# Blaizzy/mlx-audio

Measured on AMD Instinct MI355X. Metric: audio samples/sec + real-time factor, Kokoro-82M TTS, higher is better.
Workload: dtype bf16 weights x fp32 activations: vocoder convs = fp16 hi pass (v_mfma_f32_32x32x16_f16) + block-scaled FP4 (e2m1) lo pass (v_mfma_scale_f32_32x32x64_f8f6f4 cbsz / blgp 4, OCP MX: E8M0 scale per row x 32 channels / per output column), fp32 accumulate; front end bf16 hi+lo split; 1 GPU; Kokoro-82M bf16 TTS, tokens->waveform, canonical short sentence T=80 F=264 (6.6 s @ 24 kHz); utterances_per_gpu=64, global_batch=64, samples_per_utterance=158400, parallelism=utterance-dp1, precision_mode=6, wire=fp32

## Files before the change

include/mi355audio.h:

```cpp
#ifndef MI355AUDIO_H
#define MI355AUDIO_H

#include <stdint.h>

#ifdef __cplusplus
extern "C" {
#endif

#define MI355_OK 0
#define MI355_ERR_ARG (-1)
#define MI355_ERR_LAUNCH (-2)
#define MI355_ERR_UNSUPPORTED (-3)

const char* mi355_last_error(void);
int mi355_abi_version(void);
int mi355_device_info(int dev, char* name, int name_cap, int* cu_count, int* lds_bytes);

enum { MI355_ACT_NONE = 0, MI355_ACT_LEAKY = 1, MI355_ACT_SNAKE = 2, MI355_ACT_GELU = 3,
       MI355_ACT_ELU = 4,
       MI355_ACT_SILU = 5,
       MI355_ACT_GELU_TANH = 6,
       MI355_ACT_TANH = 7 };

typedef struct {
// ... 265 lines not shown
  int32_t pre_tanh;
  float* y; int64_t y_bstride; int32_t ldy;
  int32_t B; int32_t T; int32_t C; int32_t pad;
} mi355_ecapa_rows_args;
int mi355_ecapa_rows(const mi355_ecapa_rows_args* a, void* stream);
typedef struct {
  const float* x; int64_t x_bstride; int32_t ldx;
  int32_t B; int32_t T; int32_t C;
  float eps;
  float* mean; float* std; int32_t out_ld;
} mi355_time_moments_args;
int mi355_time_moments(const mi355_time_moments_args* a, void* stream);
typedef struct {
  const float* x; int64_t x_bstride; int32_t ldx;
  const float* logits; int64_t l_bstride; int32_t ldl;
  int32_t B; int32_t T; int32_t C;
  float eps;
  float* out; int32_t out_ld;
} mi355_attentive_pool_args;
int mi355_attentive_pool(const mi355_attentive_pool_args* a, void* stream);

typedef struct {
  const float* x; int64_t x_bstride; int32_t ldx; int32_t C; int32_t L; const int32_t* lens; int32_t B;
  const float* up_filter; const float* down_filter;
  const float* alpha; const float* inv_beta;
  float* y; int64_t y_bstride; int32_t ldy;
} mi355_aa_act_args;
int mi355_aa_activation(const mi355_aa_act_args* a, void* stream);

typedef struct {
  const float* x; int64_t x_bstride; int32_t n_in; int32_t rows;
  const double* table; int32_t up; int32_t down; int32_t K; int32_t first;
  float* y; int64_t y_bstride; int32_t n_out;
} mi355_resample_args;
int mi355_resample_poly(const mi355_resample_args* a, void* stream);

typedef struct {
  const float* x; int64_t x_bstride; int32_t ldx; int32_t C; int32_t L; const int32_t* lens; int32_t B;
  const float* scale; const float* shift; int32_t pre_ld; float slope;
  const float* w;
  const float* bias;
  float* y; int64_t y_bstride; int32_t ldy;
} mi355_pool_up2_args;
int mi355_adain_pool_up2(const mi355_pool_up2_args* a, void* stream);

typedef struct {
  const float* x; int64_t x_rstride; int32_t W; int64_t rows;
  int32_t size; int32_t mode; int32_t align_corners; float scale; float half_scale;
  float* y; int64_t y_rstride;
} mi355_interp1d_args;
int mi355_interpolate1d(const mi355_interp1d_args* a, void* stream);

int mi355_conv1d_c1_k3s2(const float* x, int32_t ldx_b, int32_t Lin, const int32_t* lens_in,
                         float w0, float w1, float w2, float bias, float* y, int64_t y_bstride, int32_t ldy, int32_t col,
                         int32_t Lout, int32_t B, void* stream);

typedef struct {
  const float* f0; int32_t ld_f0; int32_t L2; const int32_t* lens2; int32_t B;
  int32_t up; int32_t H; float sr; float sine_amp; float noise_std; float voiced_thr;
  const float* rand_ini; const float* noise;
  const float* lin_w; float lin_b;
  float* phase_ws;
  float* out; int32_t ld_out;
  float* quant_ws;
  int32_t coarse_f32;
} mi355_sine_source_args;
int mi355_sine_source(const mi355_sine_source_args* a, void* stream);

typedef struct {
  const float* x; int32_t ldx; int32_t L; const int32_t* lens; int32_t B;
  int32_t n_fft; int32_t hop; const float* window;
  float* y; int64_t y_bstride; int32_t ldy;
} mi355_stft_magphase_args;
int mi355_stft_magphase(const mi355_stft_magphase_args* a, void* stream);

typedef struct {
  const float* x; int64_t x_bstride; int32_t ldx; int32_t Fr; const int32_t* lens; int32_t B;
  int32_t n_fft; int32_t hop; const float* window;
  float* audio; int32_t ld_audio;
} mi355_istft_head_args;
int mi355_istft_head(const mi355_istft_head_args* a, void* stream);

typedef struct {
  const float* x; int32_t ldx; int32_t L; int32_t B;
  int32_t n_fft; int32_t hop; const float* window;
  int32_t pad_mode; int32_t n_frames;
  float* out;
} mi355_stft_args;
int mi355_stft(const mi355_stft_args* a, void* stream);

typedef struct {
  const float* x; int32_t ldx; int32_t L; int32_t B;
  int32_t n_fft; int32_t hop; const float* window; int32_t pad_mode; int32_t n_frames;
  const float* fb; int32_t n_mels; int32_t mode;
  float* out;
  float* gmax;
  float log_guard;
} mi355_logmel_args;
int mi355_logmel(const mi355_logmel_args* a, void* stream);
int mi355_logmel_finish(float* y, int64_t n_per_item, const float* gmax, int32_t B, void* stream);

typedef struct {
  const float* x; int32_t L;
  int32_t win; int32_t shift; int32_t pad; int32_t n_fft; int32_t n_frames;
  const float* window;
  const float* noise;
  float dither; float preemph;
  float* frames;
} mi355_kaldi_frames_args;
int mi355_kaldi_frames(const mi355_kaldi_frames_args* a, void* stream);
int mi355_polar_spec(const float* x, int64_t x_bstride, int32_t ldx, int32_t Fr, int32_t nb, int32_t B, float clip, float* spec, void* stream);


typedef struct {
  const float* spec; int32_t n_frames; int32_t B;
  int32_t n_fft; int32_t hop; const float* window; const float* norm;
  int32_t norm_mode;
  int32_t clamp; int32_t trim; int32_t out_len;
  float* frames_ws;
  float* out; int32_t ld_out;
} mi355_istft_args;
int mi355_istft(const mi355_istft_args* a, void* stream);

enum { MI355_KV_F32 = 0, MI355_KV_BF16 = 1, MI355_KV_F16 = 2 };
typedef struct {
  const float* q; int64_t q_bstride; int32_t ldq;
  const float* k; int64_t k_bstride; int32_t ldk;
  const float* v; int64_t v_bstride; int32_t ldv;
  int32_t heads; int32_t kv_heads; int32_t dh;
  int32_t Tq; int32_t Tk;
  const int32_t* lens_q;
  const int32_t* lens_k;
  int32_t causal; int32_t window; float scale;
  int32_t B;
  int32_t mode;
  float* out; int64_t out_bstride; int32_t ldo;
  const int32_t* k_start;
  float* split_ws; int32_t* split_cnt; int32_t nsplit;
  int64_t k_hstride; int64_t v_hstride;
  int32_t kv_dtype;
  const float* new_k; const float* new_v; int64_t new_bstride;
  const float* q_norm_w; const float* k_norm_w; float norm_eps;
  const float* rope_cos; const float* rope_sin; int32_t rope_rows; int32_t rope_mode; int32_t rope_pos;
  int32_t in_kgroups; int64_t in_kg_stride; const float* q_bias; const float* k_bias; const float* v_bias;
  const float* q_wscale; const float* k_wscale; const float* v_wscale;
  uint16_t* out_planes; int32_t planes_R; int32_t planes_dtype;
} mi355_flash_attn_args;
int mi355_flash_attention(const mi355_flash_attn_args* a, void* stream);

typedef struct {
  const float* logits; int32_t ld; int32_t V; int32_t B;
  int32_t* tokens; int32_t tokens_ld; int32_t n;
  int32_t sample_begin;
  const float* suppress_mask;
  const int32_t* blank_ids; int32_t n_blank;
  int32_t timestamp_rules;
  int32_t timestamp_begin; int32_t eot; int32_t no_timestamps;
  int32_t max_initial_timestamp_index;
  const float* gumbel; float temperature;
  float* sum_logprobs;
  float* filtered;
  const int32_t* forced_next;
  float* split_ws; int32_t* split_cnt;
} mi355_whisper_step_args;
int mi355_whisper_greedy_step(const mi355_whisper_step_args* a, void* stream);
int mi355_softmax_prob_at(const float* logits, int32_t ld, int32_t V, int32_t B, int32_t token, float* out, void* stream);
// ... 284 lines not shown
```

mlx_audio_amd/csrc/source.hip:

```cpp
#include "block_reduce.h"

namespace {

#pragma clang fp contract(off)

__device__ __forceinline__ float mul_rn(float a, float b) { return a * b; }
__device__ __forceinline__ float add_rn(float a, float b) { return a + b; }
__device__ __forceinline__ float sub_rn(float a, float b) { return a - b; }

__device__ __forceinline__ void lin_coord(int i, float scale, float half_scale, int in_w, int& lo, int& hi, float& fr) {
  float x = mul_rn((float)i, scale);
  x = add_rn(x, half_scale);
  x = sub_rn(x, 0.5f);
  x = fmaxf(x, 0.0f);
  lo = (int)floorf(x);
  hi = min(lo + 1, in_w - 1);
  fr = sub_rn(x, (float)lo);
}

struct SineDims { int L; int small; int big; float sc_dn, hsc_dn, sc_up, hsc_up; };

__host__ __device__ inline SineDims sine_dims(int len2, int up, int coarse_f32) {
  SineDims d;
  d.L = len2 * up;
// ... 194 lines not shown
    const int j = i / N, n = i - j * N;
    const float* sp = spec + j * nb * 2;
    double acc = (double)sp[0];
    if ((N & 1) == 0) acc += ((n & 1) ? -1.0 : 1.0) * (double)sp[(nb - 1) * 2];
    const int kend = (N & 1) ? nb : nb - 1;
    int m = n;
    for (int k = 1; k < kend; ++k) {
      acc += 2.0 * ((double)sp[k * 2] * twc[m] - (double)sp[k * 2 + 1] * tws[m]);
      m += n; if (m >= N) m -= N;
    }
    td[i] = mul_rn((float)(acc / (double)N), win[n]);
  }
  __syncthreads();
  const int total = (Fr - 1) * hop;
  for (int i = threadIdx.x; i < kHeadFrames * hop; i += blockDim.x) {
    const int p = blockIdx.x * kHeadFrames * hop + i;
    const int t = p - N / 2;
    if (t < 0 || t >= total) continue;
    int f_lo = (p - N + hop) / hop; if (p - N + 1 <= 0) f_lo = 0;
    int f_hi = p / hop; if (f_hi > Fr - 1) f_hi = Fr - 1;
    float rec = 0.f, ws = 0.f;
    for (int f = f_lo; f <= f_hi; ++f) {
      const int n = p - f * hop;
      if (n < 0 || n >= N) continue;
      rec = add_rn(rec, td[(f - fa) * N + n]);
      ws = add_rn(ws, mul_rn(win[n], win[n]));
    }
    a.audio[(int64_t)b * a.ld_audio + t] = (ws > 1e-10f) ? rec / ws : rec;
  }
}

struct SmallTw { double c[32]; double s[32]; };

template <int N, int HOP>
__global__ __launch_bounds__(256) void stft_magphase_fast_kernel(const mi355_stft_magphase_args a, const SmallTw tw) {
  constexpr int nb = N / 2 + 1, FB = 256, SPAN = (FB - 1) * HOP + N, YS = 2 * nb + 1;
  __shared__ float xs[SPAN];
  __shared__ float ys[FB * YS];
  const int b = blockIdx.y, tid = threadIdx.x;
  const int len = a.lens ? a.lens[b] : a.L;
  const int nframes = len / HOP + 1;
  const int f0 = blockIdx.x * FB;
  if (f0 >= nframes) return;
  const float* xb = a.x + (int64_t)b * a.ldx;
  for (int j = tid; j < SPAN; j += 256) {
    int i = f0 * HOP + j - N / 2;
    if (i < 0) i = -i;
    if (i >= len) i = 2 * (len - 1) - i;
    i = i < 0 ? 0 : (i >= len ? len - 1 : i);
    xs[j] = xb[i];
  }
  __syncthreads();
  double xw[N];
#pragma unroll
  for (int n = 0; n < N; ++n) xw[n] = (double)mul_rn(xs[tid * HOP + n], a.window[n]);
  double sp[N / 2], sm[N / 2];
#pragma unroll
  for (int n = 1; n < N / 2; ++n) { sp[n] = xw[n] + xw[N - n]; sm[n] = xw[n] - xw[N - n]; }
  float* yrow = ys + tid * YS;
#pragma unroll
  for (int k = 0; k < nb; ++k) {
    double re = (k & 1) ? xw[0] - xw[N / 2] : xw[0] + xw[N / 2];
    double im = 0.0;
#pragma unroll
    for (int n = 1; n < N / 2; ++n) {
      const int m = (k * n) % N;
      re = fma(sp[n], tw.c[m], re);
      im = fma(-sm[n], tw.s[m], im);
    }
    const float ref = (float)re;
    const float imf = (k == 0 || 2 * k == N) ? 0.0f : (float)im;
    yrow[k] = hypotf(ref, imf);
    yrow[nb + k] = atan2f(imf, ref);
  }
  __syncthreads();
  float* yb = a.y + (int64_t)b * a.y_bstride;
  const int nrows = min(FB, nframes - f0);
  for (int i = tid; i < nrows * 2 * nb; i += 256) {
    const int r = i / (2 * nb), c = i - r * (2 * nb);
    yb[(int64_t)(f0 + r) * a.ldy + c] = ys[r * YS + c];
  }
}

template <int N, int HOP>
__global__ __launch_bounds__(256) void istft_head_fast_kernel(const mi355_istft_head_args a, const SmallTw tw) {
  constexpr int nb = N / 2 + 1, HALO = (N + HOP - 1) / HOP, FT = 256, FO = FT - HALO, XS = 2 * nb + 1, TS = N + 1;
  __shared__ float xin[FT * XS];
  __shared__ float td[FT * TS];
  const int b = blockIdx.y, tid = threadIdx.x;
  const int Fr = a.lens ? a.lens[b] : a.Fr;
  const int fa = blockIdx.x * FO - HALO;
  const float* xb = a.x + (int64_t)b * a.x_bstride;
  for (int i = tid; i < FT * 2 * nb; i += 256) {
    const int j = i / (2 * nb), c = i - j * (2 * nb), f = fa + j;
    xin[j * XS + c] = (f >= 0 && f < Fr) ? xb[(int64_t)f * a.ldx + c] : 0.f;
  }
  __syncthreads();
  {
    const int f = fa + tid;
    const bool valid = f >= 0 && f < Fr;
    const float* xr = xin + tid * XS;
    double re[nb], im[nb];
#pragma unroll
    for (int k = 0; k < nb; ++k) {
      const float mag = expf(xr[k]);
      const float ph = sinf(xr[nb + k]);
      float sn, cs;
      sincosf(ph, &sn, &cs);
      re[k] = valid ? (double)mul_rn(mag, cs) : 0.0;
      im[k] = valid ? (double)mul_rn(mag, sn) : 0.0;
    }
    float* tr = td + tid * TS;
#pragma unroll
    for (int n = 0; n <= N / 2; ++n) {
      const double base = (n & 1) ? re[0] - re[nb - 1] : re[0] + re[nb - 1];
      double A = 0.0, Bs = 0.0;
#pragma unroll
      for (int k = 1; k < nb - 1; ++k) {
        const int m = (k * n) % N;
        A = fma(re[k], tw.c[m], A);
        Bs = fma(im[k], tw.s[m], Bs);
      }
      constexpr double inv_n = 1.0 / (double)N;
      tr[n] = mul_rn((float)((base + 2.0 * (A - Bs)) * inv_n), a.window[n]);
      if (n > 0 && n < N / 2) tr[N - n] = mul_rn((float)((base + 2.0 * (A + Bs)) * inv_n), a.window[N - n]);
    }
  }
  __syncthreads();
  const int total = (Fr - 1) * HOP;
  for (int i = tid; i < FO * HOP; i += 256) {
    const int p = blockIdx.x * FO * HOP + i;
    const int t = p - N / 2;
    if (t < 0 || t >= total) continue;
    int f_lo = (p - N + HOP) / HOP; if (p - N + 1 <= 0) f_lo = 0;
    int f_hi = p / HOP; if (f_hi > Fr - 1) f_hi = Fr - 1;
    float rec = 0.f, ws = 0.f;
    for (int f = f_lo; f <= f_hi; ++f) {
      const int n = p - f * HOP;
      if (n < 0 || n >= N) continue;
      rec = add_rn(rec, td[(f - fa) * TS + n]);
      const float w = a.window[n];
      ws = add_rn(ws, mul_rn(w, w));
    }
    a.audio[(int64_t)b * a.ld_audio + t] = (ws > 1e-10f) ? rec / ws : rec;
  }
}

SmallTw make_small_tw(int N) {
  SmallTw tw;
  for (int m = 0; m < 32; ++m) {
    const long double ang = 2.0L * 3.14159265358979323846264338327950288L * (long double)(m % N) / (long double)N;
    tw.c[m] = (double)cosl(ang);
    tw.s[m] = (double)sinl(ang);
  }
  for (int m = 0; m < N; ++m) {
    if ((4 * m) % N == 0) {
      const int q = (4 * m) / N;
      tw.c[m] = q == 0 ? 1.0 : (q == 2 ? -1.0 : 0.0);
      tw.s[m] = q == 1 ? 1.0 : (q == 3 ? -1.0 : 0.0);
    }
  }
  return tw;
}

__global__ __launch_bounds__(256) void interpolate1d_kernel(const mi355_interp1d_args a) {
  const int64_t i = (int64_t)blockIdx.x * 256 + threadIdx.x;
  if (i >= a.rows * (int64_t)a.size) return;
  const int64_t r = i / a.size;
  const int o = (int)(i - r * a.size);
  const float* xr = a.x + r * a.x_rstride;
  float* yr = a.y + r * a.y_rstride;
  const int W = a.W;
  if (a.mode == 0) {
    int idx = a.size == 1 ? 0 : (int)floorf(((float)o * a.scale));
    idx = idx < 0 ? 0 : (idx > W - 1 ? W - 1 : idx);
    yr[o] = xr[idx];
    return;
  }
  if (W == 1) { yr[o] = xr[0]; return; }
  float x;
  if (a.align_corners && a.size > 1) x = ((float)o * a.scale);
  else if (a.size == 1) x = 0.f;
  else {
    x = ((float)o * a.scale);
    if (!a.align_corners) {
      x = x + a.half_scale;
      x = x - 0.5f;
      x = fmaxf(x, 0.f);
    }
  }
  const int lo = (int)floorf(x);
  const int hi = lo + 1 < W - 1 ? lo + 1 : W - 1;
  const float frac = x - (float)lo;
  const float lo_term = xr[lo < W ? lo : W - 1] * (1.0f - frac);
  const float hi_term = xr[hi] * frac;
  yr[o] = lo_term + hi_term;
}

__device__ __forceinline__ float fq_prologue(const mi355_fake_quant_args& a, float t, int b, int c) {
  if (a.pre_scale) t = t * a.pre_scale[(int64_t)b * a.pre_ld + c] + a.pre_shift[(int64_t)b * a.pre_ld + c];
  if (a.pre_act == MI355_ACT_LEAKY) t = t > 0.f ? t : t * a.pre_slope;
  else if (a.pre_act == MI355_ACT_SNAKE) {
    const float al = a.pre_alpha[c];
    const float sn = sinf(al * t);
    t = t + (1.0f / al) * (sn * sn);
  }
  return t;
}

template <bool VEC>
__global__ __launch_bounds__(256) void fq_prepare_kernel(const mi355_fake_quant_args a) {
  const int b = blockIdx.y;
  const int len = a.lens ? a.lens[b] : a.L;
  const float* xb = a.x + (int64_t)b * a.x_bstride;
  float* yb = a.y + (int64_t)b * a.y_bstride;
  float nmn = 0.f, mx = 0.f;
  if (VEC) {
    const int C4 = a.C >> 2, rps = C4 >= 256 ? 1 : 256 / C4, span = C4 >= 256 ? 256 : C4;
    const int ty = C4 >= 256 ? 0 : (int)threadIdx.x / C4, tx = (int)threadIdx.x - ty * span;
    for (int l = blockIdx.x * rps + ty; l < len && ty < rps; l += gridDim.x * rps) {
      for (int c4 = tx; c4 < C4; c4 += span) {
        const float4 v = *(const float4*)(xb + (int64_t)l * a.ldx + 4 * c4);
        float4 t;
        t.x = fq_prologue(a, v.x, b, 4 * c4);
        t.y = fq_prologue(a, v.y, b, 4 * c4 + 1);
        t.z = fq_prologue(a, v.z, b, 4 * c4 + 2);
        t.w = fq_prologue(a, v.w, b, 4 * c4 + 3);
        *(float4*)(yb + (int64_t)l * a.ldy + 4 * c4) = t;
// ... 60 lines not shown
  MI355_CLEAR_ERROR();
  if (vec) {
    const int c4 = a.C / 4, rps = c4 >= 256 ? 1 : 256 / c4;
    const unsigned nblk = (unsigned)std::max<int64_t>(1, std::min<int64_t>(((int64_t)a.L + 8 * rps - 1) / (8 * rps), 4096 / std::max(1, a.B) + 1));
    hipLaunchKernelGGL(fq_prepare_kernel<true>, dim3(nblk, a.B), dim3(256), 0, st, a);
    MI355_LAUNCH_CHECK("fake_quant_u8 (prepare)");
    hipLaunchKernelGGL(fq_apply_kernel<true>, dim3(nblk, a.B), dim3(256), 0, st, a);
    MI355_LAUNCH_CHECK("fake_quant_u8 (apply)");
    return MI355_OK;
  }
  const unsigned nblk = (unsigned)std::min<int64_t>((n + 1023) / 1024, 1024);
  hipLaunchKernelGGL(fq_prepare_kernel<false>, dim3(nblk, a.B), dim3(256), 0, st, a);
  MI355_LAUNCH_CHECK("fake_quant_u8 (prepare)");
  hipLaunchKernelGGL(fq_apply_kernel<false>, dim3(nblk, a.B), dim3(256), 0, st, a);
  MI355_LAUNCH_CHECK("fake_quant_u8 (apply)");
  return MI355_OK;
}

extern "C" int mi355_sine_source(const mi355_sine_source_args* ap, void* stream) {
  MI355_REQUIRE(ap && ap->f0 && ap->rand_ini && ap->noise && ap->lin_w && ap->phase_ws && ap->out, "sine_source: null tensor");
  const mi355_sine_source_args a = *ap;
  MI355_REQUIRE(a.H > 0 && a.H <= 64 && a.up > 0 && a.L2 > 0 && a.B > 0, "sine_source: bad shape");
  const SineDims d = sine_dims(a.L2, a.up, a.coarse_f32);
  MI355_REQUIRE(d.small <= a.L2 + 1, "sine_source: coarse length %d exceeds workspace", d.small);
  hipStream_t st = (hipStream_t)stream;
  MI355_CLEAR_ERROR();
  MI355_REQUIRE(a.H <= kMergeMaxH, "sine_source: at most %d harmonics", kMergeMaxH);
  hipLaunchKernelGGL(sine_phase_kernel, dim3(a.B), dim3(256), sizeof(float) * a.H * kPhaseChunk, st, a);
  MI355_LAUNCH_CHECK("sine_phase");
  MI355_CLEAR_ERROR();
  if (a.quant_ws) {
    hipError_t e = hipMemsetAsync(a.quant_ws, 0, sizeof(float) * 2 * a.B, st);
    MI355_REQUIRE(e == hipSuccess, "sine_source: memset failed: %s", hipGetErrorString(e));
    hipLaunchKernelGGL(sine_merge_kernel<true>, dim3((d.L + 255) / 256, a.B), dim3(256), 0, st, a);
    MI355_LAUNCH_CHECK("sine_merge (extrema)");
  }
  hipLaunchKernelGGL(sine_merge_kernel<false>, dim3((d.L + 255) / 256, a.B), dim3(256), 0, st, a);
  MI355_LAUNCH_CHECK("sine_merge");
  return MI355_OK;
}

extern "C" int mi355_stft_magphase(const mi355_stft_magphase_args* ap, void* stream) {
  MI355_REQUIRE(ap && ap->x && ap->window && ap->y, "stft_magphase: null tensor");
  const mi355_stft_magphase_args a = *ap;
  MI355_REQUIRE(a.n_fft >= 2 && a.n_fft <= kMaxSmallFft, "stft_magphase: n_fft must be in [2, %d]", kMaxSmallFft);
  MI355_REQUIRE(a.hop > 0 && a.L > a.n_fft / 2, "stft_magphase: input too short for reflect padding");
  const int nframes = a.L / a.hop + 1;
  MI355_CLEAR_ERROR();
  if (a.n_fft == 20 && a.hop == 5) {
    static const SmallTw tw20 = make_small_tw(20);
    hipLaunchKernelGGL((stft_magphase_fast_kernel<20, 5>), dim3((nframes + 255) / 256, a.B), dim3(256), 0, (hipStream_t)stream, a, tw20);
    MI355_LAUNCH_CHECK("stft_magphase");
    return MI355_OK;
  }
  hipLaunchKernelGGL(stft_magphase_kernel, dim3((nframes + 255) / 256, a.B), dim3(256), 0, (hipStream_t)stream, a);
  MI355_LAUNCH_CHECK("stft_magphase");
  return MI355_OK;
}

extern "C" int mi355_istft_head(const mi355_istft_head_args* ap, void* stream) {
  MI355_REQUIRE(ap && ap->x && ap->window && ap->audio, "istft_head: null tensor");
  const mi355_istft_head_args a = *ap;
  MI355_REQUIRE(a.n_fft >= 2 && a.n_fft <= kMaxSmallFft && a.hop > 0 && a.Fr > 1, "istft_head: bad shape");
  const int N = a.n_fft, nb = N / 2 + 1;
  if (N == 20 && a.hop == 5) {
    static const SmallTw tw20 = make_small_tw(20);
    constexpr int FO = 256 - (20 + 5 - 1) / 5;
    const int total_untrimmed = (a.Fr - 1) * 5 + 20;
    MI355_CLEAR_ERROR();
    hipLaunchKernelGGL((istft_head_fast_kernel<20, 5>), dim3((total_untrimmed + FO * 5 - 1) / (FO * 5), a.B), dim3(256), 0, (hipStream_t)stream, a, tw20);
    MI355_LAUNCH_CHECK("istft_head");
    return MI355_OK;
  }
  const int halo = (N + a.hop - 1) / a.hop, FT = kHeadFrames + halo;
  const size_t lds = sizeof(double) * 2 * N + sizeof(float) * N + sizeof(float) * FT * nb * 2 + sizeof(float) * FT * N;
  const int total_untrimmed = (a.Fr - 1) * a.hop + N;
  const int blocks = (total_untrimmed + kHeadFrames * a.hop - 1) / (kHeadFrames * a.hop);
  MI355_CLEAR_ERROR();
  hipLaunchKernelGGL(istft_head_kernel, dim3(blocks, a.B), dim3(256), lds, (hipStream_t)stream, a);
  MI355_LAUNCH_CHECK("istft_head");
  return MI355_OK;
}

extern "C" int mi355_interpolate1d(const mi355_interp1d_args* ap, void* stream) {
  MI355_REQUIRE(ap && ap->x && ap->y, "interpolate1d: null tensor");
  const mi355_interp1d_args a = *ap;
  MI355_REQUIRE(a.rows > 0 && a.W >= 1 && a.size >= 1 && (a.mode == 0 || a.mode == 1), "interpolate1d: bad arguments");
  MI355_CLEAR_ERROR();
  const int64_t n = a.rows * (int64_t)a.size;
  hipLaunchKernelGGL(interpolate1d_kernel, dim3((unsigned)((n + 255) / 256)), dim3(256), 0, (hipStream_t)stream, a);
  MI355_LAUNCH_CHECK("interpolate1d");
  return MI355_OK;
}
```

mlx_audio_amd/ops.py:

```python
from __future__ import annotations

import ctypes
import math
import os
from dataclasses import dataclass
from typing import Optional, Tuple

import numpy as np
import torch

from . import _lib

ACT_NONE, ACT_LEAKY, ACT_SNAKE, ACT_GELU, ACT_ELU, ACT_SILU, ACT_GELU_TANH, ACT_TANH = 0, 1, 2, 3, 4, 5, 6, 7

PROFILE = None


def _stream() -> int:
    return torch.cuda.current_stream().cuda_stream


def profile_finalize(entries):
    torch.cuda.synchronize()
    out = []
# ... 1285 lines not shown
    raw = torch.zeros((B, T), dtype=torch.float32, device=device)
    frames = torch.empty((B,), dtype=torch.int32, device=device)
    idx = torch.zeros((B, idx_cap), dtype=torch.int32, device=device)
    kw = dict(T=T, lens=_ptr(lens), B=B, speed=speed, forced_dur=_ptr(forced), dur=_ptr(dur), dur_raw=_ptr(raw),
              frames=_ptr(frames), idx=_ptr(idx), idx_ld=idx_cap, bins=bins, max_frames=max_frames)
    if logits is not None:
        _, _, _, bs, ld = _nlc(logits)
        kw.update(logits=_ptr(logits), bstride=bs, ld=ld)
    _lib.call_struct("mi355_duration_align", "mi355_duration_args", _stream(), **kw)
    return dur, raw, frames, idx


def adain_pool_up2(x: torch.Tensor, scale, shift, slope: float, w: torch.Tensor, bias: torch.Tensor, y: torch.Tensor, lens=None):
    B, L, C, xbs, ldx = _nlc(x)
    _, _, _, ybs, ldy = _nlc(y)
    _lib.call_struct("mi355_adain_pool_up2", "mi355_pool_up2_args", _stream(), x=_ptr(x), x_bstride=xbs, ldx=ldx, C=C, L=L,
                     lens=_ptr(lens), B=B, scale=_ptr(scale), shift=_ptr(shift), pre_ld=scale.stride(0), slope=slope,
                     w=_ptr(w), bias=_ptr(bias), y=_ptr(y), y_bstride=ybs, ldy=ldy)
    return y


def aa_activation(x: torch.Tensor, y: torch.Tensor, up_filter: torch.Tensor, down_filter: torch.Tensor, alpha: torch.Tensor, inv_beta: torch.Tensor, lens=None):
    B, L, C, xbs, ldx = _nlc(x)
    _, _, _, ybs, ldy = _nlc(y)
    assert up_filter.numel() == 12 and down_filter.numel() == 12 and alpha.numel() >= C and inv_beta.numel() >= C
    _lib.call_struct("mi355_aa_activation", "mi355_aa_act_args", _stream(), x=_ptr(x), x_bstride=xbs, ldx=ldx, C=C, L=L, lens=_ptr(lens), B=B,
                     up_filter=_ptr(up_filter), down_filter=_ptr(down_filter), alpha=_ptr(alpha), inv_beta=_ptr(inv_beta), y=_ptr(y), y_bstride=ybs, ldy=ldy)
    return y


def resample_poly(x: torch.Tensor, table: torch.Tensor, up: int, down: int, first: int, n_out: int, y: Optional[torch.Tensor] = None) -> torch.Tensor:
    assert x.dim() == 2 and x.dtype == torch.float32 and x.stride(1) == 1 and table.dtype == torch.float64 and table.is_contiguous() and table.shape[1] == up
    rows, n_in = x.shape
    if y is None:
        y = torch.empty(rows, n_out, device=x.device, dtype=torch.float32)
    assert y.shape == (rows, n_out) and y.stride(1) == 1 and y.dtype == torch.float32
    _lib.call_struct("mi355_resample_poly", "mi355_resample_args", _stream(), x=_ptr(x), x_bstride=x.stride(0), n_in=n_in, rows=rows, table=_ptr(table),
                     up=up, down=down, K=table.shape[0], first=first, y=_ptr(y), y_bstride=y.stride(0), n_out=n_out)
    return y


def conv1d_c1_k3s2(x: torch.Tensor, w3, bias: float, y: torch.Tensor, col: int, lens_in=None):
    assert x.dim() == 2 and x.stride(1) == 1
    B, Lout, _, ybs, ldy = _nlc(y)
    lib = _lib.load()
    rc = lib.mi355_conv1d_c1_k3s2(_ptr(x), x.stride(0), x.shape[1], _ptr(lens_in), float(w3[0]), float(w3[1]), float(w3[2]),
                                  float(bias), _ptr(y), ybs, ldy, col, Lout, B, _stream())
    _lib.check(rc, "mi355_conv1d_c1_k3s2")
    return y


def sine_source(f0: torch.Tensor, rand_ini: torch.Tensor, noise: torch.Tensor, lin_w: torch.Tensor, lin_b: float, up: int,
                lens2=None, sr: float = 24000.0, sine_amp: float = 0.1, noise_std: float = 0.003, voiced_thr: float = 10.0, quant: bool = False,
                coarse_f32: bool = False):
    B, L2 = f0.shape
    H = rand_ini.shape[1]
    assert f0.stride(1) == 1 and noise.is_contiguous() and tuple(noise.shape) == (B, L2 * up, H)
    ws = torch.empty((B, H, L2 + 1), dtype=torch.float32, device=f0.device)
    out = torch.zeros((B, L2 * up), dtype=torch.float32, device=f0.device)
    _lib.call_struct("mi355_sine_source", "mi355_sine_source_args", _stream(), f0=_ptr(f0), ld_f0=f0.stride(0), L2=L2,
                     lens2=_ptr(lens2), B=B, up=up, H=H, sr=sr, sine_amp=sine_amp, noise_std=noise_std, voiced_thr=voiced_thr,
                     rand_ini=_ptr(rand_ini), noise=_ptr(noise), lin_w=_ptr(lin_w), lin_b=lin_b, phase_ws=_ptr(ws),
                     out=_ptr(out), ld_out=out.stride(0),
                     quant_ws=_ptr(torch.empty((B, 2), dtype=torch.float32, device=f0.device)) if quant else None, coarse_f32=int(bool(coarse_f32)))
    return out


def stft_magphase(x: torch.Tensor, n_fft: int, hop: int, window: torch.Tensor, y: torch.Tensor, lens=None):
    assert x.dim() == 2 and x.stride(1) == 1
    B, _, _, ybs, ldy = _nlc(y)
    _lib.call_struct("mi355_stft_magphase", "mi355_stft_magphase_args", _stream(), x=_ptr(x), ldx=x.stride(0), L=x.shape[1],
                     lens=_ptr(lens), B=B, n_fft=n_fft, hop=hop, window=_ptr(window), y=_ptr(y), y_bstride=ybs, ldy=ldy)
    return y


def istft_head(x: torch.Tensor, n_fft: int, hop: int, window: torch.Tensor, audio: torch.Tensor, lens=None):
    B, Fr, _, xbs, ldx = _nlc(x)
    _lib.call_struct("mi355_istft_head", "mi355_istft_head_args", _stream(), x=_ptr(x), x_bstride=xbs, ldx=ldx, Fr=Fr,
                     lens=_ptr(lens), B=B, n_fft=n_fft, hop=hop, window=_ptr(window), audio=_ptr(audio),
                     ld_audio=audio.stride(0))
    return audio


def stft_frames(x: torch.Tensor, n_fft: int, hop: int, window: torch.Tensor, pad_mode: int, n_frames: int):
    assert x.dim() == 2 and x.stride(1) == 1 and x.dtype == torch.float32
    B, L = x.shape
    out = torch.empty((B, n_frames, n_fft // 2 + 1, 2), dtype=torch.float32, device=x.device)
    _lib.call_struct("mi355_stft", "mi355_stft_args", _stream(), x=_ptr(x), ldx=x.stride(0), L=L, B=B, n_fft=n_fft, hop=hop,
                     window=_ptr(window), pad_mode=pad_mode, n_frames=n_frames, out=_ptr(out))
    return torch.view_as_complex(out)


def logmel(x: torch.Tensor, n_fft: int, hop: int, window: torch.Tensor, pad_mode: int, n_frames: int, fb: torch.Tensor,
           mode: int, log_guard: float = 0.0, fixed_max: Optional[float] = None):
    assert x.dim() == 2 and x.stride(1) == 1 and fb.is_contiguous()
    B, L = x.shape
    n_mels = fb.shape[0]
    out = torch.empty((B, n_frames, n_mels), dtype=torch.float32, device=x.device)
    gmax = torch.empty((B,), dtype=torch.float32, device=x.device) if mode == 0 else None
    _lib.call_struct("mi355_logmel", "mi355_logmel_args", _stream(), x=_ptr(x), ldx=x.stride(0), L=L, B=B, n_fft=n_fft,
                     hop=hop, window=_ptr(window), pad_mode=pad_mode, n_frames=n_frames, fb=_ptr(fb), n_mels=n_mels,
                     mode=mode, out=_ptr(out), gmax=None if fixed_max is not None else _ptr(gmax), log_guard=float(log_guard))
    if mode == 0:
        if fixed_max is not None:
            gmax.fill_(float(fixed_max))
        lib = _lib.load()
        rc = lib.mi355_logmel_finish(_ptr(out), n_frames * n_mels, _ptr(gmax), B, _stream())
        _lib.check(rc, "mi355_logmel_finish")
    return out


def kaldi_frames(x: torch.Tensor, win: int, shift: int, pad: int, n_fft: int, n_frames: int, window: torch.Tensor, preemph: float,
                 noise: Optional[torch.Tensor] = None, dither: float = 0.0) -> torch.Tensor:
    assert x.dim() == 1 and x.is_contiguous() and x.dtype == torch.float32 and window.numel() == win
    out = torch.empty((n_frames, n_fft), dtype=torch.float32, device=x.device)
    if noise is not None:
        assert noise.is_contiguous() and tuple(noise.shape) == (n_frames, win)
    _lib.call_struct("mi355_kaldi_frames", "mi355_kaldi_frames_args", _stream(), x=_ptr(x), L=x.numel(), win=win, shift=shift, pad=pad, n_fft=n_fft,
                     n_frames=n_frames, window=_ptr(window), noise=_ptr(noise), dither=dither, preemph=preemph, frames=_ptr(out))
    return out


def polar_spec(x: torch.Tensor, nb: int, clip: float = 1e2) -> torch.Tensor:
    B, Fr, C, xbs, ldx = _nlc(x)
    assert C >= 2 * nb
    spec = torch.empty((B, Fr, nb), dtype=torch.complex64, device=x.device)
    lib = _lib.load()
    rc = lib.mi355_polar_spec(_ptr(x), xbs, ldx, Fr, nb, B, float(clip), _ptr(torch.view_as_real(spec)), _stream())
    _lib.check(rc, "mi355_polar_spec")
    return spec


def istft_frames(spec: torch.Tensor, n_fft: int, hop: int, window: torch.Tensor, norm: torch.Tensor, norm_mode: int,
                 clamp: bool, trim: int, out_len: int):
    sr = torch.view_as_real(spec.contiguous())
    B, n_frames = spec.shape[0], spec.shape[1]
    ws = torch.empty((B, (n_frames + 1) // 2 * 2, n_fft), dtype=torch.float32, device=spec.device)
    out = torch.empty((B, out_len), dtype=torch.float32, device=spec.device)
    _lib.call_struct("mi355_istft", "mi355_istft_args", _stream(), spec=_ptr(sr), n_frames=n_frames, B=B, n_fft=n_fft,
                     hop=hop, window=_ptr(window), norm=_ptr(norm), norm_mode=norm_mode, clamp=int(clamp), trim=trim,
                     out_len=out_len, frames_ws=_ptr(ws), out=_ptr(out), ld_out=out.stride(0))
    return out
```

mlx_audio_amd/tts/models/kokoro/engine.py:

```python
from __future__ import annotations

import math
import os
from dataclasses import dataclass, field
from typing import Dict, List, Optional, Sequence

import numpy as np
import torch

from .... import ops
from ....ops import ACT_GELU, ACT_GELU_TANH, ACT_LEAKY, ACT_NONE, ACT_SNAKE, PackedConv, round_up


def fold_weight_norm(v: torch.Tensor, g: torch.Tensor, param_dtype: torch.dtype) -> torch.Tensor:
    v_ = v.to(param_dtype)
    g_ = g.to(param_dtype)
    axes = tuple(range(1, v_.dim()))
    nrm = torch.sqrt((v_ * v_).sum(dim=axes, keepdim=True))
    w = (v_ / (nrm + torch.tensor(1e-7, dtype=param_dtype))) * g_
    return w.to(torch.float32)


@dataclass
class _AdaIN:
# ... 614 lines not shown
        ops.conv1d_c1_k3s2(n_in, self.n_conv[0], self.n_conv[1], dec_in, hid + 1, lens_in=lens_2f)
        cd, gd, ad = self.cdim, self.gdim, self.adim
        c_cat = cd + ad + 2
        ca = self._new(B, Fm, round_up(c_cat, 32), zero=True)
        cb = self._new(B, Fm, round_up(c_cat, 32), zero=True)
        trace = {}
        self._resblk1d_fwd(self.enc_blk, dec_in[:, :, :c_in], gb_dec, ca[:, :, :cd], lens_f)
        if return_intermediates:
            trace.update(dec_in=dec_in[:, :, :c_in].clone(), enc=ca[:, :, :cd].clone())
        self._convq("decoder.asr_res.0", asr, self.asr_res, ca[:, :, cd:cd + ad], lens_in=lens_f, lens_out=lens_f, flatten=True)
        ca[:, :, cd + ad:c_cat].copy_(dec_in[:, :, hid:hid + 2])
        cb[:, :, cd:c_cat].copy_(ca[:, :, cd:c_cat])
        cur, nxt = ca, cb
        for i in range(3):
            self._resblk1d_fwd(self.dec_blks[i], cur[:, :, :c_cat], gb_dec, nxt[:, :, :cd], lens_f)
            cur, nxt = nxt, cur
            if return_intermediates:
                trace[f"dec{i}"] = cur[:, :, :cd].clone()
        xg = self._new(B, 2 * Fm, gd)
        self._resblk1d_fwd(self.dec_blks[3], cur[:, :, :c_cat], gb_dec, xg, lens_f, lens_2f)

        up = self.total_up
        L2 = 2 * Fm
        if rand_ini is None or noise is None:
            gen = torch.Generator(device=dev).manual_seed(noise_seed)
            rand_ini = torch.rand((B, 9), generator=gen, device=dev, dtype=torch.float32)
            noise = torch.randn((B, L2 * up, 9), generator=gen, device=dev, dtype=torch.float32)
        rand_ini = rand_ini.to(dev).contiguous()
        noise = noise.to(dev).contiguous()
        g_n = "decoder.generator"
        har_src = ops.sine_source(f0_curve, rand_ini, noise, self.src_w, self.src_b, up, lens2=lens_2f,
                                  quant=bool(self.qmods) and self._isq(f"{g_n}.m_source.l_linear"), coarse_f32=self.coarse_f32)
        nb2 = self.n_fft + 2
        nbp = ops.round_up(nb2, 4)
        n_har = L2 * up // self.hop + 1
        har = self._new(B, n_har, nbp, zero=True)[:, :, :nb2]
        lens_samples = frames * (2 * up) if ragged else None
        ops.stft_magphase(har_src, self.n_fft, self.hop, self.window, har, lens=lens_samples)
        if "har" in overrides:
            har.copy_(overrides["har"].to(device=dev, dtype=torch.float32))
        lens_har = lens_samples // self.hop + 1 if ragged else None
        x = xg
        L = L2
        lens_x = lens_2f
        nk = len(self.rk)
        for i, (u, k) in enumerate(zip(self.rates, self.kers)):
            last = i + 1 == len(self.rates)
            cout = self.ups[i].cout // u
            Lo = L * u + (1 if last else 0)
            lens_o = (lens_x * u + (1 if last else 0)) if ragged else None
            xsrc = self._new(B, Lo, cout)
            har_i = har
            if self.qmods and self._isq(f"{g_n}.noise_convs.{i}"):
                har_i = ops.fake_quant_u8(har, y=self._new(B, n_har, nbp, zero=True)[:, :, :nb2], lens=lens_har)
            if not last:
                sf = int(np.prod(self.rates[i + 1:]))
                self._conv(har_i, self.noise_convs[i], xsrc, lens_in=lens_har, lens_out=lens_o,
                           flat=dict(ldx=sf * nbp, x_off=-((sf + 1) // 2) * nbp, channels=nbp))
            else:
                self._conv(har_i, self.noise_convs[i], xsrc, lens_in=lens_har, lens_out=lens_o)
            if return_intermediates:
                trace[f"nconv{i}"] = xsrc.clone()
            xsrc = self._resblock1_fwd(self.noise_res[i], xsrc, gb_dec, lens_o)
            if return_intermediates:
                trace[f"nres{i}"] = xsrc.clone()
            kp = k // u
            xu = self._new(B, Lo, cout)
            lens_gemm = (lens_x + (kp - 1)) if ragged else None
            lens_ct = (lens_x * u) if ragged else None
            self._convq(f"{g_n}.ups.{i}", x, self.ups[i], xu, pad=kp - 1, lout=L + kp - 1, lens_in=lens_x, lens_out=lens_gemm, pre_act=ACT_LEAKY,
                        pre_slope=0.1, res=xsrc, up=dict(s=u, p=(k - u) // 2, cout=cout, row_off=1 if last else 0, lout=L * u, lens=lens_ct))
            if last:
                xu[:, 0, :].copy_(xsrc[:, 0, :])
            if return_intermediates:
                trace[f"xu{i}"] = xu.clone()
            acc = self._new(B, Lo, cout)
            xu_sums = torch.empty(B * cout * 2, dtype=torch.float64, device=dev)
            for j in range(nk):
                self._resblock1_fwd(self.resblocks[i * nk + j], xu, gb_dec, lens_o, out=acc, accumulate=j > 0,
                                    out_scale=(1.0 / nk) if j == nk - 1 else 1.0, x_sums=(xu_sums, j > 0))
            x, L, lens_x = acc, Lo, lens_o
            if return_intermediates:
                trace[f"stage{i}"] = acc.clone()
        post = self._new(B, L, round_up(nb2, 4))
        self._convq(f"{g_n}.conv_post", x, self.conv_post, post[:, :, :nb2], pad=3, lens_in=lens_x, lens_out=lens_x, pre_act=ACT_LEAKY, pre_slope=0.01)
        audio = self._new(B, (L - 1) * self.hop, zero=True)
        ops.istft_head(post[:, :, :nb2], self.n_fft, self.hop, self.window, audio, lens=lens_x)
        outs = [audio[b, : Fs[b] * 2 * up] for b in range(B)]
        durs = [dur[b, : Ts[b]] for b in range(B)]
        if return_intermediates:
            return outs, durs, dict(d=d, en=en, f0=f0_curve, n=n_curve, asr=asr, t_en=t_en, dur_raw=dur_raw, har_src=har_src,
                                    har=har, bert=h, xg=xg, post=post[:, :, :nb2], dec3=xg, **trace)
        return outs, durs
```

Measured before the change: 201.3 million samples/s.

## Fuse conv_post GEMM with iSTFT head into a single kernel

```diff
diff --git a/include/mi355audio.h b/include/mi355audio.h
--- a/include/mi355audio.h
+++ b/include/mi355audio.h
@@ -371,6 +371,15 @@
 int mi355_istft_head(const mi355_istft_head_args* a, void* stream);
 
 typedef struct {
+  const float* x; int64_t x_bstride; int32_t ldx; int32_t Cin; int32_t L; const int32_t* lens; int32_t B;
+  const uint16_t* w; const float* bias; int32_t Cout; int32_t K; int32_t dil; int32_t pad;
+  int32_t pre_act; float pre_slope; int32_t precision;
+  int32_t n_fft; int32_t hop; const float* window;
+  float* audio; int32_t ld_audio;
+} mi355_conv_post_istft_args;
+int mi355_conv_post_istft(const mi355_conv_post_istft_args* a, void* stream);
+
+typedef struct {
   const float* x; int32_t ldx; int32_t L; int32_t B;
   int32_t n_fft; int32_t hop; const float* window;
   int32_t pad_mode; int32_t n_frames;
diff --git a/mlx_audio_amd/csrc/source.hip b/mlx_audio_amd/csrc/source.hip
--- a/mlx_audio_amd/csrc/source.hip
+++ b/mlx_audio_amd/csrc/source.hip
@@ -300,6 +300,58 @@
   }
 }
 
+template <int N>
+__device__ __forceinline__ void head_frame_spectrum(const float* xr, const bool valid, double (&re)[N / 2 + 1], double (&im)[N / 2 + 1]) {
+  constexpr int nb = N / 2 + 1;
+#pragma unroll
+  for (int k = 0; k < nb; ++k) {
+    const float mag = expf(xr[k]);
+    const float ph = sinf(xr[nb + k]);
+    float sn, cs;
+    sincosf(ph, &sn, &cs);
+    re[k] = valid ? (double)mul_rn(mag, cs) : 0.0;
+    im[k] = valid ? (double)mul_rn(mag, sn) : 0.0;
+  }
+}
+template <int N>
+__device__ __forceinline__ void head_frame_synth(const double (&re)[N / 2 + 1], const double (&im)[N / 2 + 1], const float* window, const SmallTw& tw, float* tr) {
+  constexpr int nb = N / 2 + 1;
+#pragma unroll
+  for (int n = 0; n <= N / 2; ++n) {
+    const double base = (n & 1) ? re[0] - re[nb - 1] : re[0] + re[nb - 1];
+    double A = 0.0, Bs = 0.0;
+#pragma unroll
+    for (int k = 1; k < nb - 1; ++k) {
+      const int m = (k * n) % N;
+      A = fma(re[k], tw.c[m], A);
+      Bs = fma(im[k], tw.s[m], Bs);
+    }
+    constexpr double inv_n = 1.0 / (double)N;
+    tr[n] = mul_rn((float)((base + 2.0 * (A - Bs)) * inv_n), window[n]);
+    if (n > 0 && n < N / 2) tr[N - n] = mul_rn((float)((base + 2.0 * (A + Bs)) * inv_n), window[N - n]);
+  }
+}
+template <int N, int HOP, int FO, int TS>
+__device__ __forceinline__ void head_overlap_add(const float* td, const int fa, const int Fr, const int blk, const float* window, float* audio_b, const int tid) {
+  const int total = (Fr - 1) * HOP;
+  for (int i = tid; i < FO * HOP; i += 256) {
+    const int p = blk * FO * HOP + i;
+    const int t = p - N / 2;
+    if (t < 0 || t >= total) continue;
+    int f_lo = (p - N + HOP) / HOP; if (p - N + 1 <= 0) f_lo = 0;
+    int f_hi = p / HOP; if (f_hi > Fr - 1) f_hi = Fr - 1;
+    float rec = 0.f, ws = 0.f;
+    for (int f = f_lo; f <= f_hi; ++f) {
+      const int n = p - f * HOP;
+      if (n < 0 || n >= N) continue;
+      rec = add_rn(rec, td[(f - fa) * TS + n]);
+      const float w = window[n];
+      ws = add_rn(ws, mul_rn(w, w));
+    }
+    audio_b[t] = (ws > 1e-10f) ? rec / ws : rec;
+  }
+}
+
 template <int N, int HOP>
 __global__ __launch_bounds__(256) void istft_head_fast_kernel(const mi355_istft_head_args a, const SmallTw tw) {
   constexpr int nb = N / 2 + 1, HALO = (N + HOP - 1) / HOP, FT = 256, FO = FT - HALO, XS = 2 * nb + 1, TS = N + 1;
@@ -316,52 +368,148 @@
   __syncthreads();
   {
     const int f = fa + tid;
-    const bool valid = f >= 0 && f < Fr;
-    const float* xr = xin + tid * XS;
     double re[nb], im[nb];
-#pragma unroll
-    for (int k = 0; k < nb; ++k) {
-      const float mag = expf(xr[k]);
-      const float ph = sinf(xr[nb + k]);
-      float sn, cs;
-      sincosf(ph, &sn, &cs);
-      re[k] = valid ? (double)mul_rn(mag, cs) : 0.0;
-      im[k] = valid ? (double)mul_rn(mag, sn) : 0.0;
-    }
-    float* tr = td + tid * TS;
-#pragma unroll
-    for (int n = 0; n <= N / 2; ++n) {
-      const double base = (n & 1) ? re[0] - re[nb - 1] : re[0] + re[nb - 1];
-      double A = 0.0, Bs = 0.0;
-#pragma unroll
-      for (int k = 1; k < nb - 1; ++k) {
-        const int m = (k * n) % N;
-        A = fma(re[k], tw.c[m], A);
-        Bs = fma(im[k], tw.s[m], Bs);
+    head_frame_spectrum<N>(xin + tid * XS, f >= 0 && f < Fr, re, im);
+    head_frame_synth<N>(re, im, a.window, tw, td + tid * TS);
+  }
+  __syncthreads();
+  head_overlap_add<N, HOP, FO, TS>(td, fa, Fr, blockIdx.x, a.window, a.audio + (int64_t)b * a.ld_audio, tid);
+}
+
+constexpr int kCpTaps = 7;
+
+__device__ __forceinline__ void lds_only_barrier() {
+  asm volatile("s_waitcnt lgkmcnt(0)" ::: "memory");
+  __builtin_amdgcn_s_barrier();
+  asm volatile("" ::: "memory");
+}
+
+template <int N, int HOP>
+__global__ __launch_bounds__(256) void conv_post_istft_kernel(const mi355_conv_post_istft_args a, const SmallTw tw) {
+  constexpr int nb = N / 2 + 1, HALO = (N + HOP - 1) / HOP, FT = 256, FO = FT - HALO, XS = 2 * nb + 1, TS = N + 1;
+  constexpr int K = kCpTaps, PAD = (K - 1) / 2, R = FT + K - 1, NP = (R + 31) / 32, IMG = R * 64;
+  constexpr int WB = K * 2048, WPIECES = WB / 16, NWR = (WPIECES + 255) / 256;
+  constexpr int XIN_BYTES = FT * XS * 4, TD_BYTES = FT * TS * 4;
+  static_assert(2 * nb <= 32, "one 32-column fragment");
+  static_assert(XIN_BYTES % 16 == 0 && XIN_BYTES + TD_BYTES <= 2 * IMG + WB, "the head's arrays reuse the window");
+  __shared__ __attribute__((aligned(16))) char smem[2 * IMG + WB];
+  char* const A_hi = smem;
+  char* const A_lo = smem + IMG;
+  char* const W_l = smem + 2 * IMG;
+  float* const xin = (float*)smem;
+  float* const td = (float*)(smem + XIN_BYTES);
+
+  const int b = blockIdx.y, tid = threadIdx.x, lane = tid & 63;
+  const int wave = __builtin_amdgcn_readfirstlane(tid >> 6);
+  const int Fr = a.lens ? min(a.lens[b], a.L) : a.L;
+  if (Fr < 2 || (int)blockIdx.x * FO > Fr) return;
+  const int fa = blockIdx.x * FO - HALO;
+  const int g0 = fa - PAD;
+  const int nch = a.Cin >> 5;
+  const int c4 = (tid & 7) * 4, prow = tid >> 3;
+  const float* xb = a.x + (int64_t)b * a.x_bstride;
+  const int64_t wstep = (int64_t)(((a.Cout + 127) >> 7) << 2) * 2048;
+  const float slope = a.pre_slope;
+
+  float4 st[NP];
+  static_assert(NWR == 4 && WPIECES > 3 * 256, "weight staging: three full passes of 256 pieces and a partial one");
+  uint4 wr0, wr1, wr2, wr3;
+  const bool wlast = tid + 3 * 256 < WPIECES;
+  auto load_chunk = [&](const int chunk) {
+    auto wsrc = [&](const int p) { return (const uint4*)((const char*)a.w + (int64_t)(chunk * K + (p >> 7)) * wstep + (p & 127) * 16); };
+    wr0 = *wsrc(tid);
+    wr1 = *wsrc(tid + 256);
+    wr2 = *wsrc(tid + 512);
+    wr3 = *wsrc(wlast ? tid + 768 : tid);
+#pragma unroll
+    for (int i = 0; i < NP; ++i) {
+      int g = g0 + prow + 32 * i;
+      g = g < 0 ? 0 : (g >= a.L ? a.L - 1 : g);
+      st[i] = *(const float4*)(xb + (int64_t)g * a.ldx + chunk * 32 + c4);
+    }
+  };
+  auto stage_chunk = [&]() {
+    *(uint4*)(W_l + tid * 16) = wr0;
+    *(uint4*)(W_l + (tid + 256) * 16) = wr1;
+    *(uint4*)(W_l + (tid + 512) * 16) = wr2;
+    if (wlast) *(uint4*)(W_l + (tid + 768) * 16) = wr3;
+#pragma unroll
+    for (int i = 0; i < NP; ++i) {
+      const int r = prow + 32 * i;
+      if (r >= R) continue;
+      const int g = g0 + r;
+      const bool rowok = g >= 0 && g < Fr;
+      const float v[4] = {st[i].x, st[i].y, st[i].z, st[i].w};
+      float tt[4];
+#pragma unroll
+      for (int j = 0; j < 4; ++j) {
+        const float m = mul_rn(v[j], slope);
+        const float u = v[j] > 0.f ? v[j] : m;
+        tt[j] = rowok ? u : 0.f;
       }
-      constexpr double inv_n = 1.0 / (double)N;
-      tr[n] = mul_rn((float)((base + 2.0 * (A - Bs)) * inv_n), a.window[n]);
-      if (n > 0 && n < N / 2) tr[N - n] = mul_rn((float)((base + 2.0 * (A + Bs)) * inv_n), a.window[N - n]);
-    }
-  }
-  __syncthreads();
-  const int total = (Fr - 1) * HOP;
-  for (int i = tid; i < FO * HOP; i += 256) {
-    const int p = blockIdx.x * FO * HOP + i;
-    const int t = p - N / 2;
-    if (t < 0 || t >= total) continue;
-    int f_lo = (p - N + HOP) / HOP; if (p - N + 1 <= 0) f_lo = 0;
-    int f_hi = p / HOP; if (f_hi > Fr - 1) f_hi = Fr - 1;
-    float rec = 0.f, ws = 0.f;
-    for (int f = f_lo; f <= f_hi; ++f) {
-      const int n = p - f * HOP;
-      if (n < 0 || n >= N) continue;
-      rec = add_rn(rec, td[(f - fa) * TS + n]);
-      const float w = a.window[n];
-      ws = add_rn(ws, mul_rn(w, w));
-    }
-    a.audio[(int64_t)b * a.ld_audio + t] = (ws > 1e-10f) ? rec / ws : rec;
-  }
+      uint2 ph, pl;
+      ph.x = pack_bf16x2(tt[0], tt[1]);
+      ph.y = pack_bf16x2(tt[2], tt[3]);
+      const float h0 = __builtin_bit_cast(float, ph.x << 16), h1 = __builtin_bit_cast(float, ph.x & 0xffff0000u);
+      const float h2 = __builtin_bit_cast(float, ph.y << 16), h3 = __builtin_bit_cast(float, ph.y & 0xffff0000u);
+      pl.x = pack_bf16x2(sub_rn(tt[0], h0), sub_rn(tt[1], h1));
+      pl.y = pack_bf16x2(sub_rn(tt[2], h2), sub_rn(tt[3], h3));
+      const int addr = r * 64 + ((((c4 >> 3) ^ ((r >> 2) & 3))) << 4) + ((c4 & 4) << 1);
+      *(uint2*)(A_hi + addr) = ph;
+      *(uint2*)(A_lo + addr) = pl;
+    }
+  };
+
+  f32x16 acc[2];
+#pragma unroll
+  for (int mf = 0; mf < 2; ++mf)
+#pragma unroll
+    for (int r = 0; r < 16; ++r) acc[mf][r] = 0.f;
+  const int hl = lane & 31, hh = lane >> 5;
+
+  load_chunk(0);
+  for (int chunk = 0; chunk < nch; ++chunk) {
+    if (chunk > 0) lds_only_barrier();
+    stage_chunk();
+    if (chunk + 1 < nch) load_chunk(chunk + 1);
+    lds_only_barrier();
+#pragma unroll
+    for (int tap = 0; tap < K; ++tap) {
+#pragma unroll
+      for (int kk = 0; kk < 2; ++kk) {
+        const bf16x8 bf = *(const bf16x8*)(W_l + tap * 2048 + kk * 1024 + lane * 16);
+#pragma unroll
+        for (int mf = 0; mf < 2; ++mf) {
+          const int row = wave * 64 + mf * 32 + hl + tap;
+          const int addr = row * 64 + (((kk * 2 + hh) ^ ((row >> 2) & 3)) << 4);
+          const bf16x8 h = *(const bf16x8*)(A_hi + addr);
+          const bf16x8 l = *(const bf16x8*)(A_lo + addr);
+          acc[mf] = __builtin_amdgcn_mfma_f32_32x32x16_bf16(h, bf, acc[mf], 0, 0, 0);
+          acc[mf] = __builtin_amdgcn_mfma_f32_32x32x16_bf16(l, bf, acc[mf], 0, 0, 0);
+        }
+      }
+    }
+  }
+  lds_only_barrier();
+  if (hl < 2 * nb) {
+    const float bias = a.bias ? a.bias[hl] : 0.f;
+#pragma unroll
+    for (int mf = 0; mf < 2; ++mf)
+#pragma unroll
+      for (int r = 0; r < 16; ++r) {
+        const int j = wave * 64 + mf * 32 + (r & 3) + 8 * (r >> 2) + 4 * hh;
+        xin[j * XS + hl] = add_rn(acc[mf][r], bias);
+      }
+  }
+  __syncthreads();
+  {
+    const int f = fa + tid;
+    double re[nb], im[nb];
+    head_frame_spectrum<N>(xin + tid * XS, f >= 0 && f < Fr, re, im);
+    head_frame_synth<N>(re, im, a.window, tw, td + tid * TS);
+  }
+  __syncthreads();
+  head_overlap_add<N, HOP, FO, TS>(td, fa, Fr, blockIdx.x, a.window, a.audio + (int64_t)b * a.ld_audio, tid);
 }
 
 SmallTw make_small_tw(int N) {
@@ -588,6 +736,27 @@
   return MI355_OK;
 }
 
+extern "C" int mi355_conv_post_istft(const mi355_conv_post_istft_args* ap, void* stream) {
+  MI355_REQUIRE(ap && ap->x && ap->w && ap->window && ap->audio, "conv_post_istft: null tensor");
+  const mi355_conv_post_istft_args a = *ap;
+  if (!(a.Cin > 0 && a.Cin % 32 == 0 && a.K == kCpTaps && a.dil == 1 && a.pad == (kCpTaps - 1) / 2 && a.n_fft == 20 && a.hop == 5 &&
+        a.Cout == 2 * (a.n_fft / 2 + 1) && a.Cout <= 32 && a.pre_act == MI355_ACT_LEAKY && a.precision == 2)) {
+    mi355_set_error("conv_post_istft: unsupported shape (Cin=%d K=%d dil=%d pad=%d Cout=%d n_fft=%d hop=%d pre_act=%d precision=%d)", a.Cin, a.K, a.dil,
+                    a.pad, a.Cout, a.n_fft, a.hop, a.pre_act, a.precision);
+    return MI355_ERR_UNSUPPORTED;
+  }
+  MI355_REQUIRE(a.B > 0 && a.B <= 65535 && a.L > 1 && a.ldx >= a.Cin && (a.B == 1 || a.x_bstride >= (int64_t)a.L * a.ldx), "conv_post_istft: bad shape");
+  MI355_REQUIRE((a.ldx & 3) == 0 && (a.x_bstride & 3) == 0 && (((uintptr_t)a.x | (uintptr_t)a.w) & 15) == 0, "conv_post_istft: rows must be 16-byte aligned");
+  MI355_REQUIRE(a.B == 1 || a.ld_audio >= (a.L - 1) * a.hop, "conv_post_istft: audio rows shorter than (L - 1) * hop");
+  static const SmallTw tw20 = make_small_tw(20);
+  constexpr int FO = 256 - (20 + 5 - 1) / 5;
+  const int total_untrimmed = (a.L - 1) * 5 + 20;
+  MI355_CLEAR_ERROR();
+  hipLaunchKernelGGL((conv_post_istft_kernel<20, 5>), dim3((total_untrimmed + FO * 5 - 1) / (FO * 5), a.B), dim3(256), 0, (hipStream_t)stream, a, tw20);
+  MI355_LAUNCH_CHECK("conv_post_istft");
+  return MI355_OK;
+}
+
 extern "C" int mi355_interpolate1d(const mi355_interp1d_args* ap, void* stream) {
   MI355_REQUIRE(ap && ap->x && ap->y, "interpolate1d: null tensor");
   const mi355_interp1d_args a = *ap;
diff --git a/mlx_audio_amd/ops.py b/mlx_audio_amd/ops.py
--- a/mlx_audio_amd/ops.py
+++ b/mlx_audio_amd/ops.py
@@ -1391,6 +1391,33 @@
     return audio
 
 
+def conv_post_istft_eligible(pc: PackedConv, n_fft: int, hop: int, *, dil: int = 1, pad: int = 3, pre_act: int = ACT_LEAKY, precision: int = 2,
+                             pre_fq=None) -> bool:
+    return (pc.cin % 32 == 0 and pc.k == 7 and dil == 1 and pad == 3 and n_fft == 20 and hop == 5 and pc.cout == n_fft + 2 and pc.cout <= 32
+            and pre_act == ACT_LEAKY and precision == 2 and not pc.f16 and not pc.mx and pre_fq is None)
+
+
+def conv_post_istft(x: torch.Tensor, pc: PackedConv, n_fft: int, hop: int, window: torch.Tensor, audio: torch.Tensor, *, lens=None,
+                    dil: int = 1, pad: int = 3, pre_act: int = ACT_LEAKY, pre_slope: float = 0.01, precision: int = 2, pre_fq=None):
+    B, L, _, xbs, ldx = _nlc(x)
+    if conv_post_istft_eligible(pc, n_fft, hop, dil=dil, pad=pad, pre_act=pre_act, precision=precision, pre_fq=pre_fq):
+        assert audio.dim() == 2 and audio.stride(1) == 1 and audio.dtype == torch.float32 and audio.shape[1] >= (L - 1) * hop
+        if PROFILE is not None:
+            e0, e1 = torch.cuda.Event(enable_timing=True), torch.cuda.Event(enable_timing=True)
+            e0.record()
+            PROFILE.append(((L * B) if lens is None else lens.sum(), pc.cin, pc.cout, pc.k, dil, 0, e0, e1))
+        _lib.call_struct("mi355_conv_post_istft", "mi355_conv_post_istft_args", _stream(), x=_ptr(x), x_bstride=xbs, ldx=ldx, Cin=pc.cin, L=L,
+                         lens=_ptr(lens), B=B, w=_ptr(pc.w), bias=_ptr(pc.bias), Cout=pc.cout, K=pc.k, dil=dil, pad=pad, pre_act=pre_act,
+                         pre_slope=pre_slope, precision=precision, n_fft=n_fft, hop=hop, window=_ptr(window), audio=_ptr(audio),
+                         ld_audio=audio.stride(0))
+        if PROFILE is not None:
+            e1.record()
+        return audio
+    post = torch.empty((B, L, round_up(pc.cout, 4)), dtype=torch.float32, device=x.device)[:, :, :pc.cout]
+    conv_gemm(x, pc, post, dil=dil, pad=pad, lens_in=lens, lens_out=lens, pre_act=pre_act, pre_slope=pre_slope, precision=precision, pre_fq=pre_fq)
+    return istft_head(post, n_fft, hop, window, audio, lens=lens)
+
+
 def stft_frames(x: torch.Tensor, n_fft: int, hop: int, window: torch.Tensor, pad_mode: int, n_frames: int):
     assert x.dim() == 2 and x.stride(1) == 1 and x.dtype == torch.float32
     B, L = x.shape
diff --git a/mlx_audio_amd/tts/models/kokoro/engine.py b/mlx_audio_amd/tts/models/kokoro/engine.py
--- a/mlx_audio_amd/tts/models/kokoro/engine.py
+++ b/mlx_audio_amd/tts/models/kokoro/engine.py
@@ -720,10 +720,14 @@
             x, L, lens_x = acc, Lo, lens_o
             if return_intermediates:
                 trace[f"stage{i}"] = acc.clone()
-        post = self._new(B, L, round_up(nb2, 4))
-        self._convq(f"{g_n}.conv_post", x, self.conv_post, post[:, :, :nb2], pad=3, lens_in=lens_x, lens_out=lens_x, pre_act=ACT_LEAKY, pre_slope=0.01)
         audio = self._new(B, (L - 1) * self.hop, zero=True)
-        ops.istft_head(post[:, :, :nb2], self.n_fft, self.hop, self.window, audio, lens=lens_x)
+        post = None
+        if not return_intermediates and not (self.qmods and self._isq(f"{g_n}.conv_post")):
+            ops.conv_post_istft(x, self.conv_post, self.n_fft, self.hop, self.window, audio, lens=lens_x, pre_slope=0.01, precision=self._prec(self.conv_post))
+        else:
+            post = self._new(B, L, round_up(nb2, 4))
+            self._convq(f"{g_n}.conv_post", x, self.conv_post, post[:, :, :nb2], pad=3, lens_in=lens_x, lens_out=lens_x, pre_act=ACT_LEAKY, pre_slope=0.01)
+            ops.istft_head(post[:, :, :nb2], self.n_fft, self.hop, self.window, audio, lens=lens_x)
         outs = [audio[b, : Fs[b] * 2 * up] for b in range(B)]
         durs = [dur[b, : Ts[b]] for b in range(B)]
         if return_intermediates:
```

Measured after the change: 203.6 million samples/s, median of 6. +1.2%, better.
